# andrewrosemberg/DiffOpt.jl

Measured on AMD Instinct MI355X. Metric: KKT sensitivity solves/sec (fwd+rev) on batched QPs, higher is better.
Workload: dtype f64; 1 GPU; config 2: dense QP batch, fwd+rev sensitivities; problems_per_gpu=1024, n=200, m_ineq=300, p_eq=0, parallelism=batch-sharded x1

## Files before the change

### diffopt.jl_amd/csrc/abi.hip

```cpp
#include <algorithm>
#include <chrono>
#include <cstdlib>
#include <cstring>
#include <initializer_list>

#include "dopt_internal.h"

using dopt::DevBuf;
using dopt::Error;
using dopt::Handle;

struct dopt_handle : public Handle {};

namespace {

template <class F>
int guarded(dopt_handle* h, F&& f) {
  if (!h) return -1;
  try {
    h->err.clear();
    DOPT_CHECK_HIP(hipSetDevice(h->device));
    return f();
  } catch (const Error& e) {
    h->err = e.msg;
// ... 92 lines not shown
  *out = nullptr;
  if (batch < 0 || n < 0 || m < 0 || p < 0 ||
      (kind != DOPT_KIND_QP && kind != DOPT_KIND_CONIC && kind != DOPT_KIND_NLP))
    return -1;
  int ndev = 0;
  if (hipGetDeviceCount(&ndev) != hipSuccess || ndev <= 0) return -4;
  if (device < 0 || device >= ndev) return -1;
  auto* h = new dopt_handle();
  h->device = device;
  h->batch = batch;
  h->n = n;
  h->m = m;
  h->p = p;
  h->kind = kind;
  int rc = guarded(h, [&]() {
    DOPT_CHECK_HIP(hipStreamCreateWithFlags(&h->stream, hipStreamNonBlocking));
    h->own_stream = true;
    if (const char* e = getenv("DOPT_CONIC_SPLIT")) {
      if (e[0] == '0' || e[0] == '1') h->conic_split = e[0] - '0';
    }
    if (const char* e = getenv("DOPT_LU")) h->lu_mode = atoi(e) != 0;
    if (const char* e = getenv("DOPT_SYM")) h->sym_mode = atoi(e) != 0;
    if (const char* e = getenv("DOPT_LEFT")) h->left_mode = atoi(e) != 0;
    if (const char* e = getenv("DOPT_NLP_REDUCE")) h->nlp_reduce = atoi(e) != 0;
    if (const char* e = getenv("DOPT_SPLIT_FUSE")) h->split_fuse = atoi(e) != 0;
    if (kind == DOPT_KIND_QP) {
      if ((int64_t)n + m + p > dopt::DENSE_QP_MAX) {
        h->sparse = true;
        h->kamax.ensure(sizeof(double));
        return 0;
      }
      h->nmax = (int32_t)dopt::round_up(std::max(n + m + p, 1), 32);
      h->ld = h->nmax;
      h->K.ensure((size_t)batch * h->nmax * h->ld * sizeof(double));
      h->ipiv.ensure((size_t)batch * std::max(h->nmax, 1) * sizeof(int32_t));
      h->s.ensure((size_t)batch * std::max(m, 1) * sizeof(double));
      h->kidx.ensure((size_t)2 * batch * std::max(m, 1) * sizeof(int32_t));
      h->kls.ensure((size_t)2 * batch * std::max(m, 1) * sizeof(double));
      h->gk.ensure((size_t)batch * std::max(n, 1) * std::max(m, 1) * sizeof(double));
      h->meta.ensure((size_t)std::max<int64_t>(batch, 1) * sizeof(dopt::QPMeta));
      h->kamax.ensure((size_t)std::max<int64_t>(batch, 1) * sizeof(double));
      h->rhs.ensure((size_t)3 * batch * std::max(h->nmax, 1) * sizeof(double));
      h->x.ensure((size_t)2 * batch * std::max(h->nmax, 1) * sizeof(double));
    }
    return 0;
  });
// ... 63 lines not shown
  });
}

int dopt_set_memory(dopt_handle* h, int32_t mem) {
  return guarded(h, [&]() {
    if (mem != DOPT_MEM_HOST && mem != DOPT_MEM_DEVICE) throw Error(-1, "bad memory mode");
    h->mem = mem;
    return 0;
  });
}

int dopt_set_sparse(dopt_handle* h, int32_t on) {
  return guarded(h, [&]() {
    if (h->kind != DOPT_KIND_QP && h->kind != DOPT_KIND_CONIC) throw Error(-1, "dopt_set_sparse: QP and conic handles only");
    if (h->kind == DOPT_KIND_CONIC) {
      h->sparse = on != 0;
      h->cset = h->cfactored = false;
      return 0;
    }
    if (!on && (int64_t)h->n + h->m + h->p > dopt::DENSE_QP_MAX)
      throw Error(-1, "dopt_set_sparse: n + m + p > 8192 has only the sparse route");
    h->sparse = on != 0;
    h->set = h->factored = h->small_ready = false;
    return 0;
  });
}

int dopt_qp_set(dopt_handle* h, const double* Q, const double* G, const double* hv,
                const double* A, const double* z, const double* lam, const double* nu) {
  return guarded(h, [&]() {
    if (h->kind != DOPT_KIND_QP) throw Error(-1, "dopt_qp_set on a non-QP handle");
    if (h->sparse) throw Error(-1, "dopt_qp_set: a sparse-route handle takes the MOI matrix form (dopt_qp_set_csc)");
    const size_t B = h->batch, n = h->n, m = h->m, p = h->p;
    if (!Q || !z) throw Error(-1, "Q and z are required");
    if (m && (!G || !hv || !lam)) throw Error(-1, "G, h and lam are required when m > 0");
    if (p && (!A || !nu)) throw Error(-1, "A and nu are required when p > 0");
    h->set = false;
    h->factored = false;
    h->small_ready = false;
    h->Q = stage_in(*h, h->own_in[0], Q, B * n * n);
    h->G = m ? stage_in(*h, h->own_in[1], G, B * m * n) : nullptr;
    h->hv = m ? stage_in(*h, h->own_in[2], hv, B * m) : nullptr;
    h->A = p ? stage_in(*h, h->own_in[3], A, B * p * n) : nullptr;
    h->z = stage_in(*h, h->own_in[4], z, B * n);
    h->lam = m ? stage_in(*h, h->own_in[5], lam, B * m) : nullptr;
    h->nu = p ? stage_in(*h, h->own_in[6], nu, B * p) : nullptr;
// ... 1293 lines not shown
```

### diffopt.jl_amd/csrc/dopt_internal.h

```cpp
#pragma once
#include <hip/hip_runtime.h>

#include <cstdint>
#include <functional>
#include <string>
#include <vector>

#include "../../include/diffopt_mi355x.h"

#define DOPT_CHECK_HIP(expr)                                                   \
  do {                                                                         \
    hipError_t _e = (expr);                                                    \
    if (_e != hipSuccess) {                                                    \
      throw dopt::Error(-2, std::string(#expr) + ": " + hipGetErrorString(_e)); \
    }                                                                          \
  } while (0)

namespace dopt {

struct Error {
  int code;
  std::string msg;
  Error(int c, std::string m) : code(c), msg(std::move(m)) {}
};
// ... 116 lines not shown
  DevBuf gk;
  DevBuf dinv;
  DevBuf plist;
  DevBuf glist;
  DevBuf lsqr_ws;
  DevBuf binv;
  hipStream_t aux = nullptr;
  hipEvent_t ev_fork = nullptr, ev_join = nullptr, ev_qsym = nullptr, ev_crit = nullptr;
  hipStream_t crit = nullptr;
  int32_t left_mode = 1;
  DevBuf ukp;
  bool ukp_valid = false;
  bool u_missing = false;
  DevBuf qsy;
  bool qsym_pending = false;
  DevBuf fwdw;
  DevBuf krhs, kx, kfull;
  DevBuf mws;
  QPMeta* meta_host = nullptr;
  hipEvent_t meta_ev = nullptr;
  hipEvent_t meta_fork = nullptr;
  int32_t lu_mode = 1;
  int32_t sym_mode = 1;
  int32_t blocked_npmax = 0;
  bool has_generic = true;
  int32_t n_generic = 0;
  bool info_clear = false;
  bool has_lsqr = true;
  int32_t n_pivot = 0;
  bool set = false, factored = false;
  bool small_ready = false;
  bool sparse = false;
  bool sp_qnz = false;
  SpStore sp[2];
  DevBuf sp_tmp, sp_sort, sp_s, sp_ws, sp_info, sp_rhs;

  const double *cA = nullptr, *cb = nullptr, *cc = nullptr;
  const double *cx = nullptr, *cs = nullptr, *cy = nullptr;
  DevBuf own_cin[6];
  std::vector<int32_t> cones;
  DevBuf cone_dev;
  DevBuf vp, dpi, cwork, cinfo, cnorm;
  DevBuf cinfok;
  int32_t conic_k = 0;
  DevBuf csplit;
  int32_t conic_split = -1;
// ... 58 lines not shown
      DOPT_CHECK_HIP(hipEventElapsedTime(&ms, pe.second.first, pe.second.second));
      phase_ms[pe.first] += ms;
      phase_cnt[pe.first] += 1;
      ev_pool.push_back(pe.second.first);
      ev_pool.push_back(pe.second.second);
    }
    ev_pending.clear();
  }
};

inline void ensure_aux(Handle& h) {
  if (h.aux) return;
  int least = 0, greatest = 0;
  DOPT_CHECK_HIP(hipDeviceGetStreamPriorityRange(&least, &greatest));
  DOPT_CHECK_HIP(hipStreamCreateWithPriority(&h.aux, hipStreamNonBlocking, least));
  DOPT_CHECK_HIP(hipStreamCreateWithPriority(&h.crit, hipStreamNonBlocking, greatest));
  const unsigned fl = hipEventDisableTiming | hipEventReleaseToDevice;
  DOPT_CHECK_HIP(hipEventCreateWithFlags(&h.ev_fork, fl));
  DOPT_CHECK_HIP(hipEventCreateWithFlags(&h.ev_join, fl));
  DOPT_CHECK_HIP(hipEventCreateWithFlags(&h.ev_qsym, fl));
  DOPT_CHECK_HIP(hipEventCreateWithFlags(&h.ev_crit, fl));
  DOPT_CHECK_HIP(hipEventCreateWithFlags(&h.meta_fork, fl));
}
inline double* qsy_max(Handle& h) { return h.qsy.as<double>(); }
inline int32_t* qsy_flag(Handle& h) { return reinterpret_cast<int32_t*>(h.qsy.as<double>() + h.batch); }
inline void qsym_join(Handle& h) {
  if (!h.qsym_pending) return;
  DOPT_CHECK_HIP(hipStreamWaitEvent(h.stream, h.ev_qsym, 0));
  h.qsym_pending = false;
}

struct PhaseTimer {
  Handle& h;
  int phase;
  hipEvent_t e0 = nullptr, e1 = nullptr;
  PhaseTimer(Handle& hh, int ph) : h(hh), phase(ph) {
    if (!(h.prof >> ph & 1u)) return;
    e0 = h.take_event();
    e1 = h.take_event();
    DOPT_CHECK_HIP(hipEventRecord(e0, h.stream));
  }
  ~PhaseTimer() {
    if (!e0) return;
    if (hipEventRecord(e1, h.stream) == hipSuccess) h.ev_pending.push_back({phase, {e0, e1}});
  }
};
// ... 2 lines not shown
bool qp_small_eligible(const Handle& h);
void qp_small_reverse(Handle& h, const double* dl_dz, double* out, int32_t* flags);
void qp_small_forward(Handle& h, const FwdTangents& T, double* out);
void qp_reverse(Handle& h, const double* dl_dz, double* out);
struct CscTriple {
  const int64_t* cp[3];
  const int64_t* rv[3];
  const double* nz[3];
  double* dense[3];
  int rows[3];
};
void csc_to_dense3(Handle& h, const CscTriple& T);
void csc_to_dense(Handle& h, const int64_t* colptr, const int64_t* rowval, const double* nzval,
                  int64_t nnz, int rows, int ncols, double* dense, int* err);
void qp_reverse_grads(Handle& h, const double* rev, double* dQ, double* dq, double* dG, double* gc,
                      double* dA, double* ac);
void qp_forward(Handle& h, const double* dQ, const double* dq, const double* dG,
                const double* dh, const double* dA, const double* db, double* out);
void qp_forward_reverse(Handle& h, const double* dl_dz, const double* dQ,
                        const double* dq, const double* dG, const double* dh,
                        const double* dA, const double* db, double* out_rev,
                        double* out_fwd);
void qp_nopiv_factor(Handle& h, double* dinv, double* w0 = nullptr, double* w1 = nullptr);
void qp_blocked_factor(Handle& h, double* dinv, const int32_t* plist, int count);
void qp_nopiv_materialize_u(Handle& h);
void qp_blocked_solve(Handle& h, const double* dinv, int trans, const double* rhs, double* x, int sel);
void qp_blocked_solve_pair(Handle& h, const double* dinv, const double* rhs0, const double* rhs1, double* x0,
                           double* x1, int sel);
void qp_blocked_solve_multi(Handle& h, const double* dinv, int trans, int k, const double* rhs, double* x,
                            int sel);
void qp_reverse_k(Handle& h, int k, const double* dl_dz, double* out);
void qp_params_reverse(Handle& h, const double* rev, int nparam, int64_t nterms, const int32_t* t_param,
                       const int32_t* t_kind, const int32_t* t_index, const double* t_coef, double* out);
void qp_params_forward(Handle& h, const double* dp, int nparam, int64_t nterms, const int32_t* t_param,
                       const int32_t* t_kind, const int32_t* t_index, const double* t_coef, double* dq,
                       double* dh, double* db);
void qp_forward_k(Handle& h, int k, const double* dQ, const double* dq, const double* dG, const double* dh,
                  const double* dA, const double* db, double* out);
void qp_blocked_solve2(Handle& h, const double* dinv, const double* rhs_rev, const double* rhs_fwd,
                       double* x_rev, double* x_fwd, int sel, const double* w_rev = nullptr,
                       const double* w_fwd = nullptr);
size_t dinv_stride(int nmax);
using ReasmFn = std::function<void(const int32_t*, int)>;
void factor_dense(Handle& h, const ReasmFn& reasm, const std::function<void()>* pre_copy = nullptr,
                  bool* deferred = nullptr);
void factor_dense_finish(Handle& h, const ReasmFn& reasm);
// ... 54 lines not shown
```

### diffopt.jl_amd/csrc/qp.hip

```cpp
#include "device_prims.h"
#include "lsqr_core.h"
#include "qp_assemble.h"

namespace dopt {

constexpr int TPB = 256;
constexpr int OUT_LCAP = 4096;
constexpr int NB = 32;

__global__ __launch_bounds__(TPB) void qp_lu_generic_kernel(
    double* __restrict__ K, int32_t* __restrict__ ipiv, QPMeta* __restrict__ meta,
    int nmax, int ld, const int32_t* __restrict__ plist) {
  __shared__ double redv[4];
  __shared__ int redi[4];
  const int b = plist[blockIdx.x], t = threadIdx.x;
  const int lane = t & 63, wv = t >> 6;
  const int N = meta[b].nsys;
  double* Kb = K + (size_t)b * nmax * ld;
  int32_t* piv = ipiv + (size_t)b * nmax;
  int info = 0;
  for (int j = 0; j < N; ++j) {
    double best = -1.0;
    int bi = 0x7fffffff;
    for (int r = j + t; r < N; r += TPB) {
// ... 192 lines not shown
};

__global__ __launch_bounds__(TPB) void qp_lsqr_kernel(
    const double* __restrict__ K, const QPMeta* __restrict__ meta, int nmax,
    int ld, int trans, const double* __restrict__ rhs, double* __restrict__ xout,
    double* __restrict__ work) {
  __shared__ double red[4];
  const int b = blockIdx.x, t = threadIdx.x;
  if (!meta[b].iterative) return;
  const int N = meta[b].nsys;
  const double* Kb = K + (size_t)b * nmax * ld;
  double* x = work + (size_t)b * 5 * nmax;
  double* u = x + N;
  double* v = u + N;
  double* w = v + N;
  double* tmp = w + N;
  const DenseKKT op{Kb, ld, N, trans};
  LsqrScalars st;
  lsqr_solve<TPB, block_sum>(st, op, rhs + (size_t)b * nmax, 0.0, N, x, u, v, w, tmp, N, red);
  __syncthreads();
  for (int i = t; i < N; i += TPB) xout[(size_t)b * nmax + i] = x[i];
}

__global__ __launch_bounds__(TPB) void qp_rev_rhs_kernel(
    const double* __restrict__ dl_dz, const QPMeta* __restrict__ meta, int n,
    int nmax, double* __restrict__ rhs, double* __restrict__ rhs2) {
  const int b = blockIdx.x, t = threadIdx.x;
  const int N = meta[b].nsys;
  for (int i = t; i < N; i += TPB) {
    const double v = (i < n) ? dl_dz[(size_t)b * n + i] : 0.0;
    rhs[(size_t)b * nmax + i] = v;
    if (rhs2) rhs2[(size_t)b * nmax + i] = v;
  }
}

__global__ __launch_bounds__(TPB) void qp_fwd_rhs_kernel(
    const double* __restrict__ dQ, const double* __restrict__ dq,
    const double* __restrict__ dG, const double* __restrict__ dh,
    const double* __restrict__ dA, const double* __restrict__ db,
    const double* __restrict__ z, const double* __restrict__ lam,
    const double* __restrict__ nu, const int32_t* __restrict__ rpos,
    const QPMeta* __restrict__ meta, int n, int m, int p, int nmax, int zcap,
    double* __restrict__ full, double* __restrict__ rhs, double* __restrict__ rhs2) {
  extern __shared__ __attribute__((aligned(16))) double smem[];
  const int b = blockIdx.x, t = threadIdx.x, lane = t & 63, wv = t >> 6;
  const double* zg = z + (size_t)b * n;
  const double* lb = lam + (size_t)b * m;
  const double* nb = nu + (size_t)b * p;
  const bool staged = n <= zcap;
  if (staged)
    for (int i = t; i < n; i += TPB) smem[i] = zg[i];
  __syncthreads();
  const double* zs = staged ? smem : zg;
  double* r = full + (size_t)b * nmax;
  for (int i = t; i < n; i += TPB) {
    double acc = 0.0;
    if (dQ) {
      const double* Qb = dQ + (size_t)b * n * n;
      for (int j = 0; j < n; ++j) acc = fma(Qb[i + (size_t)j * n], zs[j], acc);
    }
    if (dq) acc += dq[(size_t)b * n + i];
    r[i] = acc;
  }
  __syncthreads();
  if (dG && m > 0) {
    const double* Gb = dG + (size_t)b * m * n;
    for (int i = wv; i < n; i += 4) {
      double acc = 0.0;
// ... 28 lines not shown
      for (int j = 0; j < n; ++j) az = fma(Ab[e + (size_t)j * p], zs[j], az);
    }
    r[n + m + e] = az - (db ? db[(size_t)b * p + e] : 0.0);
  }
  __syncthreads();
  const int nk = meta[b].nk;
  double* rb = rhs + (size_t)b * nmax;
  double* rb2 = rhs2 ? rhs2 + (size_t)b * nmax : nullptr;
  for (int i = t; i < n; i += TPB) {
    rb[i] = r[i];
    if (rb2) rb2[i] = r[i];
  }
  for (int l = t; l < m; l += TPB) {
    const int kk = rpos[(size_t)b * m + l];
    if (kk >= 0) {
      rb[n + kk] = r[n + l];
      if (rb2) rb2[n + kk] = r[n + l];
    }
  }
  for (int e = t; e < p; e += TPB) {
    rb[n + nk + e] = r[n + m + e];
    if (rb2) rb2[n + nk + e] = r[n + m + e];
  }
}

#ifndef DOPT_QP_NT
#define DOPT_QP_NT 0
#endif
__global__ __launch_bounds__(TPB) void qp_output_kernel(
    const double* __restrict__ x0, const double* __restrict__ G,
    const double* __restrict__ s, const int32_t* __restrict__ rpos,
    const QPMeta* __restrict__ meta, const double* __restrict__ full, int n,
    int m, int p, int nmax, int zcap, int trans0, double* __restrict__ out0, const double* __restrict__ x1,
    double* __restrict__ out1, int B) {
  extern __shared__ __attribute__((aligned(16))) double smem[];
  __shared__ int nel;
  const bool second = x1 && (int)blockIdx.x >= B;
  const int b = second ? (int)blockIdx.x - B : (int)blockIdx.x, t = threadIdx.x;
  const double* __restrict__ x = second ? x1 : x0;
  double* __restrict__ out = second ? out1 : out0;
  const int trans = second ? 1 : trans0;
  const int nk = meta[b].nk;
  const double* xb = x + (size_t)b * nmax;
  double* ob = out + (size_t)b * (n + m + p);
  const bool staged = n <= zcap;
  const double* xz = staged ? smem : xb;
// ... 195 lines not shown
static double* dinv_of(Handle& h) {
  h.dinv.ensure((size_t)h.batch * dinv_stride(h.nmax) * sizeof(double));
  return h.dinv.as<double>();
}

static QPIn qp_inputs(Handle& h) {
  static const double dummy = 0.0;
  QPIn P;
  P.Q = h.Q;
  P.G = h.m ? h.G : &dummy;
  P.h = h.m ? h.hv : &dummy;
  P.A = h.p ? h.A : &dummy;
  P.z = h.z;
  P.lam = h.m ? h.lam : &dummy;
  P.nu = h.p ? h.nu : &dummy;
  P.n = h.n;
  P.m = h.m;
  P.p = h.p;
  return P;
}

static int32_t* rpos_of(Handle& h) { return h.kidx.as<int32_t>() + (size_t)h.batch * h.m; }

template <class F>
static void prep_assemble(Handle& h, const int32_t* plist, int count, bool full, F&& after_prep) {
  if (count == 0) return;
  const QPIn P = qp_inputs(h);
  if (!full && h.n > 0) {
    ensure_aux(h);
    h.qsy.ensure((size_t)h.batch * (sizeof(double) + sizeof(int32_t)));
    DOPT_CHECK_HIP(hipEventRecord(h.ev_fork, h.stream));
    DOPT_CHECK_HIP(hipStreamWaitEvent(h.aux, h.ev_fork, 0));
    DOPT_CHECK_HIP(hipMemsetAsync(h.qsy.p, 0, h.qsy.bytes, h.aux));
    hipLaunchKernelGGL(qp_qsym_kernel, dim3((unsigned)qsym_pairs(h.n), (unsigned)count), dim3(256), 0, h.aux, P,
                       qsy_max(h), qsy_flag(h), plist);
    check_launch();
    DOPT_CHECK_HIP(hipEventRecord(h.ev_qsym, h.aux));
    h.qsym_pending = true;
  }
  const dim3 pg(count), pb(prep_threads(h.m));
  if (prep_rows_per_thread(h.m) == 2)
    hipLaunchKernelGGL(qp_prep_kernel<2>, pg, pb, prep_lds(h.n), h.stream, P, h.s.as<double>(),
                       h.kidx.as<int32_t>(), rpos_of(h), h.kls.as<double>(), h.gk.as<double>(), h.batch, h.meta.as<QPMeta>(),
                       plist, h.kamax.as<double>(), h.sym_mode);
  else
    hipLaunchKernelGGL(qp_prep_kernel<1>, pg, pb, prep_lds(h.n), h.stream, P, h.s.as<double>(),
                       h.kidx.as<int32_t>(), rpos_of(h), h.kls.as<double>(), h.gk.as<double>(), h.batch, h.meta.as<QPMeta>(),
                       plist, h.kamax.as<double>(), h.sym_mode);
  check_launch();
  after_prep();
  hipLaunchKernelGGL(qp_asm_tile_kernel, dim3((unsigned)count * ASM_WPP), dim3(512), 0, h.stream, P,
                     h.kidx.as<int32_t>(), h.kls.as<double>(), h.gk.as<double>(), h.batch, h.meta.as<QPMeta>(),
                     h.K.as<double>(), h.ld,
                     h.nmax, plist, full ? 1 : 0, h.kamax.as<double>());
  check_launch();
}
static void prep_assemble(Handle& h, const int32_t* plist, int count) { prep_assemble(h, plist, count, true, [] {}); }

static void meta_copy(Handle& h) {
  if (!h.meta_host) {
    DOPT_CHECK_HIP(hipHostMalloc((void**)&h.meta_host, std::max<size_t>(h.batch, 1) * sizeof(QPMeta)));
    DOPT_CHECK_HIP(hipEventCreateWithFlags(&h.meta_ev, hipEventDisableTiming));
  }
  DOPT_CHECK_HIP(hipMemcpyAsync(h.meta_host, h.meta.p, h.batch * sizeof(QPMeta), hipMemcpyDeviceToHost,
                                h.stream));
  DOPT_CHECK_HIP(hipEventRecord(h.meta_ev, h.stream));
}

static void meta_copy_side(Handle& h) {
  ensure_aux(h);
  if (!h.meta_host) {
    DOPT_CHECK_HIP(hipHostMalloc((void**)&h.meta_host, std::max<size_t>(h.batch, 1) * sizeof(QPMeta)));
    DOPT_CHECK_HIP(hipEventCreateWithFlags(&h.meta_ev, hipEventDisableTiming));
  }
  DOPT_CHECK_HIP(hipEventRecord(h.meta_fork, h.stream));
  DOPT_CHECK_HIP(hipStreamWaitEvent(h.crit, h.meta_fork, 0));
  DOPT_CHECK_HIP(hipMemcpyAsync(h.meta_host, h.meta.p, h.batch * sizeof(QPMeta), hipMemcpyDeviceToHost, h.crit));
  DOPT_CHECK_HIP(hipEventRecord(h.meta_ev, h.crit));
}

static void meta_sizes(Handle& h) {
  DOPT_CHECK_HIP(hipEventSynchronize(h.meta_ev));
  int npmax = 0;
  h.has_generic = h.has_lsqr = false;
  for (int64_t b = 0; b < h.batch; ++b) {
    const QPMeta& mm = h.meta_host[b];
    const int r = qp_route(mm.iterative, mm.nsys);
    if (r == ROUTE_BLOCKED) npmax = std::max(npmax, (mm.nsys + 31) & ~31);
    h.has_generic |= r == ROUTE_GENERIC;
    h.has_lsqr |= r == ROUTE_LSQR;
  }
  h.blocked_npmax = npmax;
}

static int pivot_fallback(Handle& h, const ReasmFn& reasm) {
  DOPT_CHECK_HIP(hipEventSynchronize(h.meta_ev));
  std::vector<int32_t> list;
  for (int64_t b = 0; b < h.batch; ++b)
    if (h.meta_host[b].lu == LU_REJECT && ((h.meta_host[b].nsys + 31) & ~31) <= PIVOT_MAX)
      list.push_back((int32_t)b);
  const int count = (int)list.size();
  if (count) {
    h.plist.ensure(list.size() * sizeof(int32_t));
    DOPT_CHECK_HIP(hipMemcpyAsync(h.plist.p, list.data(), list.size() * sizeof(int32_t),
                                  hipMemcpyHostToDevice, h.stream));
    const int32_t* pl = h.plist.as<int32_t>();
    reasm(pl, count);
    qp_blocked_factor(h, dinv_of(h), pl, count);
    DOPT_CHECK_HIP(hipStreamSynchronize(h.stream));
  }
  return count;
}

static void generic_lu(Handle& h, const std::vector<int32_t>& list) {
  h.n_generic = (int)list.size();
// ... 21 lines not shown
    }
    if (any) {
      PhaseTimer pt(h, DOPT_PHASE_QP_LU_PIVOT);
      h.n_pivot = pivot_fallback(h, reasm);
    }
    if (!big.empty()) {
      h.plist.ensure(big.size() * sizeof(int32_t));
      DOPT_CHECK_HIP(hipMemcpyAsync(h.plist.p, big.data(), big.size() * sizeof(int32_t), hipMemcpyHostToDevice,
                                    h.stream));
      reasm(h.plist.as<int32_t>(), (int)big.size());
      DOPT_CHECK_HIP(hipStreamSynchronize(h.stream));
      glist.insert(glist.end(), big.begin(), big.end());
    }
  }
  h.n_generic = 0;
  if (!glist.empty()) {
    PhaseTimer pt(h, DOPT_PHASE_QP_LU_PIVOT);
    generic_lu(h, glist);
  }
}

template <class F>
static void factor_blocked(Handle& h, F&& spec, double* w0, double* w1, const ReasmFn& reasm,
                           const std::function<void()>* pre_copy = nullptr, bool* deferred = nullptr) {
  auto np_of = [](const QPMeta& mm) { return (mm.nsys + 31) & ~31; };
  std::vector<int32_t> glist;
  if (h.has_generic)
    for (int64_t b = 0; b < h.batch; ++b) {
      const QPMeta& mm = h.meta_host[b];
      if (qp_route(mm.iterative, mm.nsys) == ROUTE_GENERIC) glist.push_back((int32_t)b);
    }
  if (deferred) *deferred = false;
  if (h.lu_mode == 1) {
    {
      PhaseTimer pt(h, DOPT_PHASE_QP_LU);
      qp_nopiv_factor(h, dinv_of(h), w0, w1);
    }
    if (pre_copy) (*pre_copy)();
    if (h.blocked_npmax) meta_copy_side(h);
    spec();
    h.n_pivot = 0;
    if (deferred && h.blocked_npmax && glist.empty()) {
      *deferred = true;
      return;
    }
    factor_blocked_rest(h, reasm, glist, true);
  } else {
    {
      PhaseTimer pt(h, DOPT_PHASE_QP_LU_PIVOT);
      qp_blocked_factor(h, dinv_of(h), nullptr, (int)h.batch);
    }
    spec();
    h.n_pivot = -1;
    if (h.blocked_npmax > PIVOT_MAX)
      for (int64_t b = 0; b < h.batch; ++b) {
        const QPMeta& mm = h.meta_host[b];
        if (qp_route(mm.iterative, mm.nsys) == ROUTE_BLOCKED && np_of(mm) > PIVOT_MAX) glist.push_back((int32_t)b);
// ... 85 lines not shown
static void finish_pair(Handle& h, double* out_rev, double* out_fwd) {
  finish_into(h, 1, rhs_of(h, 1), x_of(h, 1), full_of(h), nullptr, nullptr, nullptr, true);
  finish_into(h, 0, rhs_of(h, 0), x_of(h, 0), full_of(h), out_rev, x_of(h, 1), out_fwd);
}

static void rev_rhs(Handle& h, const double* dl_dz, double* copy = nullptr) {
  PhaseTimer pt(h, DOPT_PHASE_QP_RHS);
  hipLaunchKernelGGL(qp_rev_rhs_kernel, dim3(h.batch), dim3(TPB), 0, h.stream, dl_dz, h.meta.as<QPMeta>(),
                     h.n, h.nmax, rhs_of(h, 0), copy);
  check_launch();
}

static void fwd_rhs_into(Handle& h, const FwdTangents& T, double* full, double* rhs, double* copy = nullptr) {
  const int B = (int)h.batch, n = h.n, m = h.m, p = h.p;
  static const double dummy = 0.0;
  hipLaunchKernelGGL(qp_fwd_rhs_kernel, dim3(B), dim3(TPB), (size_t)std::min(n, ZCAP) * sizeof(double),
                     h.stream, T.dQ, T.dq, T.dG, T.dh, T.dA, T.db, h.z, m ? h.lam : &dummy,
                     p ? h.nu : &dummy, rpos_of(h), h.meta.as<QPMeta>(), n, m, p, h.nmax, ZCAP, full, rhs, copy);
  check_launch();
}
static void fwd_rhs(Handle& h, const FwdTangents& T, double* copy = nullptr) {
  PhaseTimer pt(h, DOPT_PHASE_QP_RHS);
  fwd_rhs_into(h, T, full_of(h), rhs_of(h, 1), copy);
}

static FwdTangents tangents(Handle& h, const double* dQ, const double* dq, const double* dG,
                            const double* dh, const double* dA, const double* db) {
  FwdTangents T;
  T.dQ = dQ;
  T.dq = dq;
  T.dG = h.m ? dG : nullptr;
  T.dh = h.m ? dh : nullptr;
  T.dA = h.p ? dA : nullptr;
  T.db = h.p ? db : nullptr;
  return T;
}

void qp_reverse(Handle& h, const double* dl_dz, double* out) {
  if (!h.factored) qp_factor(h);
  rev_rhs(h, dl_dz);
  {
    PhaseTimer pt(h, DOPT_PHASE_QP_SOLVE);
    qp_blocked_solve(h, dinv_of(h), 0, rhs_of(h, 0), x_of(h, 0), LU_SEL_ALL);
  }
  finish(h, 0, out);
}
// ... 88 lines not shown
  }
  solve_k(h, 1, k, rk, xk, fk, out);
}

void qp_reverse_grads(Handle& h, const double* rev, double* dQ, double* dq, double* dG, double* gc,
                      double* dA, double* ac) {
  if (!h.set) throw Error(-1, "dopt_qp_reverse_grads: dopt_qp_set has not been called");
  static const double dummy = 0.0;
  const long long per = (long long)h.n * h.n + (long long)(h.m + h.p) * h.n + h.n + h.m + h.p;
  const int gx = (int)std::max<long long>(1, std::min<long long>((per + TPB - 1) / TPB, 64));
  const int gy = (int)std::min<int64_t>(h.batch, 65535);
  hipLaunchKernelGGL(qp_reverse_grads_kernel, dim3(gx, gy), dim3(TPB), 0, h.stream, rev, h.z,
                     h.m ? h.lam : &dummy, h.p ? h.nu : &dummy, (int)h.batch, h.n, h.m, h.p, dQ, dq,
                     h.m ? dG : nullptr, h.m ? gc : nullptr, h.p ? dA : nullptr, h.p ? ac : nullptr);
  check_launch();
}

void qp_forward_reverse(Handle& h, const double* dl_dz, const double* dQ,
                        const double* dq, const double* dG, const double* dh,
                        const double* dA, const double* db, double* out_rev,
                        double* out_fwd) {
  if (!h.set) throw Error(-1, "dopt_qp_forward_reverse: dopt_qp_set has not been called");
  const FwdTangents T = tangents(h, dQ, dq, dG, dh, dA, db);
  {
    PhaseTimer pt(h, DOPT_PHASE_QP_ASSEMBLE);
    prep_assemble(h, nullptr, (int)h.batch, h.lu_mode == 0, [&] { meta_copy_side(h); });
  }
  double *w0 = nullptr, *w1 = nullptr;
  if (h.lu_mode == 1) {
    const size_t len = (size_t)h.batch * h.nmax;
    h.fwdw.ensure(2 * len * sizeof(double));
    w0 = h.fwdw.as<double>();
    w1 = w0 + len;
  }
  rev_rhs(h, dl_dz, w0);
  fwd_rhs(h, T, w1);
  meta_sizes(h);
  if (!h.blocked_npmax) w0 = w1 = nullptr;
  auto solve2 = [&](int sel, const double* sw0, const double* sw1) {
    PhaseTimer pt(h, DOPT_PHASE_QP_SOLVE);
    qp_blocked_solve2(h, dinv_of(h), rhs_of(h, 0), rhs_of(h, 1), x_of(h, 0), x_of(h, 1), sel, sw0, sw1);
  };
  const bool spec_out = h.lu_mode == 1 && !h.has_generic && !h.has_lsqr;
  h.n_generic = 0;
  factor_blocked(
      h,
      [&] {
        solve2(h.lu_mode == 1 ? LU_SEL_NOPIV : LU_SEL_ALL, w0, w1);
        if (spec_out) finish_pair(h, out_rev, out_fwd);
      },
      w0, w1, qp_reasm(h));
  if (h.n_pivot > 0) solve2(LU_SEL_PIVOT, nullptr, nullptr);
  if (!spec_out || h.n_pivot > 0 || h.n_generic > 0) finish_pair(h, out_rev, out_fwd);
  h.factored = true;
  h.info_clear = h.lu_mode == 1 && h.n_pivot == 0 && h.n_generic == 0;
}

}
```

### diffopt.jl_amd/csrc/qp_nopiv.hip

```cpp
#include "device_prims.h"
#include "nlp_defs.h"

#ifndef NLU_STOP
#define NLU_STOP 99
#endif
#ifndef NLU_ROT
#define NLU_ROT (blockIdx.x & 3)
#endif
#ifdef NLU_STAMPS
__device__ unsigned long long nlu_stamps[16];
#define NLU_MARK(k)                                                              \
  do {                                                                          \
    if (threadIdx.x == 0) {                                                     \
      const unsigned long long now_ = __builtin_amdgcn_s_memtime();             \
      atomicAdd(&nlu_stamps[k], now_ - st_last_);                               \
      st_last_ = now_;                                                          \
    }                                                                           \
  } while (0)
#define NLU_MARK_INIT unsigned long long st_last_ = __builtin_amdgcn_s_memtime()
#else
#define NLU_MARK(k) do {} while (0)
#define NLU_MARK_INIT do {} while (0)
#endif
#ifdef LDIAG_STAMPS
// ... 1343 lines not shown
        if (j < t) acc = fma(S[t * SLD + j], P[j] * vec[j], acc);
      if (t < Wv) w0b[c0 + t] = fma(acc, RP[t], vec[t]);
    } else if (t < 128) {
      const int j = t - 64;
      double acc = vec[64 + j];
#pragma unroll 8
      for (int i = 0; i < NB64; ++i)
        if (i < j) acc = fma(vec[64 + i], S[j * SLD + i], acc);
      if (j < Wv) w1b[c0 + j] = acc * P[j] * RD[j];
    }
  }
  LD_MARK(10);
}

template <class SRC>
__device__ __forceinline__ void ldiag_body(
    double* S, int b, double* __restrict__ K, int ld, int nmax, int32_t* __restrict__ perm,
    double* __restrict__ dinv, size_t dstride, QPMeta* __restrict__ meta, int c0, double* __restrict__ binv,
    double* __restrict__ ukp, double* __restrict__ w0, double* __restrict__ w1, double* __restrict__ kamax,
    const double* __restrict__ kls, int n, int m, const SRC& src) {
  LD_MARK(0);
  const QPMeta mm = meta[b];
  const int Np = nlu_np(mm);
  if (c0 >= Np || mm.lu == LU_REJECT) return;
  const int Wv = min(NB64, Np - c0);
  const int t = threadIdx.x, lane = t & 63, wv = t >> 6, g = lane >> 4, l16 = lane & 15;
  double* Kb = K + (size_t)b * nmax * ld;
  const auto sv = src_bind(src, b, mm);
  const PScale ps = pscale(kls, b, n, m, mm);
  double* ud = ukp + (size_t)b * nmax;
  double* w0b = w0 ? w0 + (size_t)b * nmax : nullptr;
  double* w1b = w0 ? w1 + (size_t)b * nmax : nullptr;
  double amax = __hip_atomic_load(kamax + b, __ATOMIC_RELAXED, __HIP_MEMORY_SCOPE_AGENT);
  if (c0 == 0) {
    if (src.qflag) {
      if (src.qflag[b]) {
        if (t == 0) meta[b].lu = LU_REJECT;
        return;
      }
      amax = fmax(amax, src.qmax[b]);
      if (t == 0) kamax[b] = amax;
    }
  }
  d4 accd[3];
#pragma unroll
  for (int q = 0; q < 3; ++q) accd[q] = (d4){0, 0, 0, 0};
  double sweep = 0.0;
// ... 125 lines not shown
  const int oq = c * n + r, og = c * v.m + rn, oa = c * v.p + (rn - nk);
  int off = cq ? (rq ? oq : (rg ? og : oa)) : rn;
  const double* base = cq ? (rq ? v.Q : (rg ? v.gk : v.A)) : v.sk;
  off = live ? off : 0;
  base = live ? base : v.Q;
  p = base + off;
  return live ? 1 : 0;
}
__device__ __forceinline__ int src_ref_tile(const NSrcB& v, const double* X, int r, int c, int ri, int ci,
                                            const double*& p) {
  const int* tc = lc_codes(X);
  return nlp_R_ref_lower(v.s->d, v.s->in, v.s->R, v.b, r, c, tc[ri], tc[64 + ci], p);
}

template <class SRC>
__device__ __forceinline__ void lcol_body(double* X, int b, int it, double* __restrict__ K, int ld, int nmax,
                                          QPMeta* __restrict__ meta, int c0, const double* __restrict__ binv,
                                          const double* __restrict__ ukp, int cnt,
                                          const double* __restrict__ kamax, const double* __restrict__ kls, int n,
                                          int m, const SRC& src) {
  const QPMeta mm = meta[b];
  const int Np = nlu_np(mm);
  const int r0 = c0 + NB64 + 64 * it;
  if (mm.lu == LU_REJECT || it >= cnt || r0 >= Np) return;
  const int sw = min(NB64, Np - r0);
  const int t = threadIdx.x, lane = t & 63, wv = t >> 6, g = lane >> 4, l16 = lane & 15;
  const bool wact = 16 * wv < sw;
  double* Kb = K + (size_t)b * nmax * ld;
  const double* ud = ukp + (size_t)b * nmax;
  const double* Bg = binv + (size_t)b * BSTR;
  const auto sv = src_bind(src, b, mm);
  const PScale ps = pscale(kls, b, n, m, mm);
  const int rho = lane >> 3, gam = lane & 7;
  auto issue = [&](int st) {
    double* buf = X + (st & 1) * LC_STAGE;
    const int ks = 16 * st;
#pragma unroll
    for (int q = 0; q < 2; ++q) {
      const int c = 2 * wv + q, r = 8 * c + rho, col = ks + 2 * (gam ^ ((r >> 1) & 7));
      const int rt = r < sw ? r0 + r : r0;
      glds16(Kb + (size_t)rt * ld + col, buf + c * 128);
      glds16(Kb + (size_t)(c0 + r) * ld + col, buf + LC_IMG + c * 128);
    }
    if (wv == 0) glds16(ud + ks + 2 * gam, X + LC_DS + (st & 1) * 128);
  };
  auto issue_uinv = [&]() {
    const int hr = lane >> 5, gq = lane & 31;
// ... 162 lines not shown

__global__ __launch_bounds__(256) void nlu_sym_uinv_kernel(double* __restrict__ dinv, size_t dstride,
                                                           const QPMeta* __restrict__ meta,
                                                           const double* __restrict__ ukp, int nmax,
                                                           const double* __restrict__ kls, int n, int m) {
  const int b = blockIdx.y, kb = blockIdx.x;
  const QPMeta mm = meta[b];
  if (mm.lu != LU_NOPIV || !mm.sym) return;
  const int Np = nlu_np(mm);
  if (32 * kb >= Np) return;
  double* D = dinv + (size_t)b * dstride + (size_t)kb * DBLK;
  const double* ud = ukp + (size_t)b * nmax + 32 * kb;
  const PScale ps = pscale(kls, b, n, m, mm);
  for (int e = threadIdx.x; e < 32 * 32; e += 256) {
    const int i = e >> 5, j = e & 31;
    D[32 * 32 + e] = i <= j ? D[j * 32 + i] / (ps(32 * kb + i) * ud[j]) : 0.0;
  }
}

}

template <class SRC>
static void left_lu(Handle& h, const SRC& src, double* dinv, double* w0, double* w1, const double* kls,
                    double* kamax) {
  const int npmax = h.blocked_npmax;
  const int B = (int)h.batch;
  const size_t dstride = dinv_stride(h.nmax);
  double* K = h.K.as<double>();
  int32_t* perm = h.ipiv.as<int32_t>();
  QPMeta* meta = h.meta.as<QPMeta>();
  h.binv.ensure((size_t)2 * B * BSTR * sizeof(double));
  h.ukp.ensure((size_t)B * h.nmax * sizeof(double));
  h.ukp_valid = true;
  h.u_missing = true;
  double* ukp = h.ukp.as<double>();
  hipStream_t S = h.stream;
  auto binv_of = [&](int c0) { return h.binv.as<double>() + (size_t)((c0 / NB64) & 1) * B * BSTR; };
  for (int c0 = 0; c0 < npmax; c0 += NB64) {
    double* bv = binv_of(c0);
    hipLaunchKernelGGL((nlu_ldiag_kernel<SRC>), dim3(B), dim3(PNT), 0, S, K, h.ld, h.nmax, perm, dinv, dstride, meta,
                       c0, bv, ukp, w0, w1, kamax, kls, h.n, h.m, src, 0);
    DOPT_CHECK_HIP(hipGetLastError());
    const int ntile = (npmax - c0 - NB64 + 63) / 64;
    if (ntile <= 0) break;
    const long long tot = (long long)ntile * B;
    if (tot > 0x7fffffffLL) throw Error(-1, "no-pivot LU: grid too large");
    hipLaunchKernelGGL((nlu_lcol_kernel<SRC>), dim3((unsigned)tot), dim3(256), 0, S, K, h.ld, h.nmax, meta, c0, bv,
                       ukp, ntile, (int)tot, kamax, kls, h.n, h.m, src);
    DOPT_CHECK_HIP(hipGetLastError());
  }
}

void qp_nopiv_factor(Handle& h, double* dinv, double* w0, double* w1) {
  qsym_join(h);
  h.ukp_valid = false;
  h.u_missing = false;
  const int npmax = h.blocked_npmax;
  if (npmax == 0) return;
  const int B = (int)h.batch;
  const bool qp = h.kind == DOPT_KIND_QP;
  const double* kls = qp ? h.kls.as<double>() : nullptr;
  double* kamax = h.kamax.as<double>();
  int lower = qp && h.meta_host ? 1 : 0;
  static const double zero = 0.0;
  QSrc src;
  src.Q = qp ? h.Q : &zero;
  src.gk = qp ? h.gk.as<double>() : &zero;
  src.kls = qp ? h.kls.as<double>() : &zero;
  src.A = qp && h.p ? h.A : &zero;
  const bool qchk = qp && h.qsy.p && h.n > 0;
  src.qmax = qchk ? qsy_max(h) : nullptr;
  src.qflag = qchk ? qsy_flag(h) : nullptr;
  src.n = h.n;
  src.m = h.m;
  src.p = h.p;
  src.B = h.batch;
  const int srcmode = qp ? 1 : 0;
  if (lower)
    for (int64_t b = 0; b < h.batch; ++b) {
      const QPMeta& mm = h.meta_host[b];
      if (qp_route(mm.iterative, mm.nsys) == ROUTE_BLOCKED && !mm.sym) {
        lower = 0;
        break;
      }
    }
  const size_t dstride = dinv_stride(h.nmax);
  double* K = h.K.as<double>();
  int32_t* perm = h.ipiv.as<int32_t>();
  QPMeta* meta = h.meta.as<QPMeta>();
  if (h.kind == DOPT_KIND_NLP && h.nlp_left) {
    NSrc ns;
    ns.d = nlp_dims(h);
    ns.in = nlp_inputs(h);
    ns.R = nlp_red_of(h);
    ns.qmax = qsy_max(h);
    ns.qflag = qsy_flag(h);
    left_lu(h, ns, dinv, w0, w1, nullptr, kamax);
    return;
  }
  if (lower && h.left_mode) {
    left_lu(h, src, dinv, w0, w1, kls, kamax);
    return;
  }
  h.binv.ensure((size_t)2 * B * BSTR * sizeof(double));
  auto binv_of = [&](int c) { return h.binv.as<double>() + (size_t)((c / NB64) & 1) * B * BSTR; };
  auto grid = [](long long g) {
    if (g > 0x7fffffffLL) throw Error(-1, "no-pivot LU: grid too large");
    return dim3((unsigned)g);
  };
  hipStream_t S = h.stream, T = h.stream;
  if (lower) {
    ensure_aux(h);
    T = h.aux;
    if (h.crit) {
      S = h.crit;
      DOPT_CHECK_HIP(hipEventRecord(h.ev_crit, h.stream));
      DOPT_CHECK_HIP(hipStreamWaitEvent(S, h.ev_crit, 0));
    }
  }
  auto fork = [&] {
    DOPT_CHECK_HIP(hipEventRecord(h.ev_fork, S));
    DOPT_CHECK_HIP(hipStreamWaitEvent(T, h.ev_fork, 0));
  };
  auto join = [&] {
// ... 93 lines not shown
```

Before: 904,800 solves/s.

## Speculatively launch left-looking LU before host metadata scan using prior call's size

Records the padded system size and symmetry status from previous forward+reverse calls. On later calls it queues prep, a fused forward/reverse RHS kernel, and the left-looking no-pivot LU before the host synchronises on the metadata copy, so the host wait no longer serialises the factor launch. If the scan shows the guess was wrong or a system is non-symmetric, it synchronises all streams and redoes the normal path. The separate rev/fwd RHS launches are also merged into one kernel with a 2B grid. This risks wasted work on misprediction and relies on the LU kernels skipping non-symmetric systems.

Result: no change. 908,400 solves/s, median of 6 (+0.4%).

```diff
diff --git a/diffopt.jl_amd/csrc/abi.hip b/diffopt.jl_amd/csrc/abi.hip
--- a/diffopt.jl_amd/csrc/abi.hip
+++ b/diffopt.jl_amd/csrc/abi.hip
@@ -138,6 +138,7 @@
     if (const char* e = getenv("DOPT_LU")) h->lu_mode = atoi(e) != 0;
     if (const char* e = getenv("DOPT_SYM")) h->sym_mode = atoi(e) != 0;
     if (const char* e = getenv("DOPT_LEFT")) h->left_mode = atoi(e) != 0;
+    if (const char* e = getenv("DOPT_LU_SPEC")) h->lu_spec = atoi(e) != 0;
     if (const char* e = getenv("DOPT_NLP_REDUCE")) h->nlp_reduce = atoi(e) != 0;
     if (const char* e = getenv("DOPT_SPLIT_FUSE")) h->split_fuse = atoi(e) != 0;
     if (kind == DOPT_KIND_QP) {
@@ -247,6 +248,7 @@
       throw Error(-1, "dopt_set_sparse: n + m + p > 8192 has only the sparse route");
     h->sparse = on != 0;
     h->set = h->factored = h->small_ready = false;
+    dopt::spec_drop(*h);
     return 0;
   });
 }
diff --git a/diffopt.jl_amd/csrc/dopt_internal.h b/diffopt.jl_amd/csrc/dopt_internal.h
--- a/diffopt.jl_amd/csrc/dopt_internal.h
+++ b/diffopt.jl_amd/csrc/dopt_internal.h
@@ -162,6 +162,9 @@
   hipEvent_t meta_fork = nullptr;
   int32_t lu_mode = 1;
   int32_t sym_mode = 1;
+  int32_t lu_spec = 1;
+  int32_t spec_np[4] = {0, 0, 0, 0};
+  bool spec_qual = false;
   int32_t blocked_npmax = 0;
   bool has_generic = true;
   int32_t n_generic = 0;
@@ -266,6 +269,10 @@
   DOPT_CHECK_HIP(hipEventCreateWithFlags(&h.ev_crit, fl));
   DOPT_CHECK_HIP(hipEventCreateWithFlags(&h.meta_fork, fl));
 }
+inline void spec_drop(Handle& h) {
+  for (int32_t& v : h.spec_np) v = 0;
+  h.spec_qual = false;
+}
 inline double* qsy_max(Handle& h) { return h.qsy.as<double>(); }
 inline int32_t* qsy_flag(Handle& h) { return reinterpret_cast<int32_t*>(h.qsy.as<double>() + h.batch); }
 inline void qsym_join(Handle& h) {
@@ -314,6 +321,7 @@
                         const double* dA, const double* db, double* out_rev,
                         double* out_fwd);
 void qp_nopiv_factor(Handle& h, double* dinv, double* w0 = nullptr, double* w1 = nullptr);
+void qp_nopiv_left_spec(Handle& h, double* dinv, double* w0, double* w1, int npmax);
 void qp_blocked_factor(Handle& h, double* dinv, const int32_t* plist, int count);
 void qp_nopiv_materialize_u(Handle& h);
 void qp_blocked_solve(Handle& h, const double* dinv, int trans, const double* rhs, double* x, int sel);
diff --git a/diffopt.jl_amd/csrc/qp.hip b/diffopt.jl_amd/csrc/qp.hip
--- a/diffopt.jl_amd/csrc/qp.hip
+++ b/diffopt.jl_amd/csrc/qp.hip
@@ -238,10 +238,10 @@
   for (int i = t; i < N; i += TPB) xout[(size_t)b * nmax + i] = x[i];
 }
 
-__global__ __launch_bounds__(TPB) void qp_rev_rhs_kernel(
-    const double* __restrict__ dl_dz, const QPMeta* __restrict__ meta, int n,
+__device__ __forceinline__ void rev_rhs_body(
+    int b, const double* __restrict__ dl_dz, const QPMeta* __restrict__ meta, int n,
     int nmax, double* __restrict__ rhs, double* __restrict__ rhs2) {
-  const int b = blockIdx.x, t = threadIdx.x;
+  const int t = threadIdx.x;
   const int N = meta[b].nsys;
   for (int i = t; i < N; i += TPB) {
     const double v = (i < n) ? dl_dz[(size_t)b * n + i] : 0.0;
@@ -249,17 +249,21 @@
     if (rhs2) rhs2[(size_t)b * nmax + i] = v;
   }
 }
-
-__global__ __launch_bounds__(TPB) void qp_fwd_rhs_kernel(
-    const double* __restrict__ dQ, const double* __restrict__ dq,
+__global__ __launch_bounds__(TPB) void qp_rev_rhs_kernel(
+    const double* __restrict__ dl_dz, const QPMeta* __restrict__ meta, int n,
+    int nmax, double* __restrict__ rhs, double* __restrict__ rhs2) {
+  rev_rhs_body(blockIdx.x, dl_dz, meta, n, nmax, rhs, rhs2);
+}
+
+__device__ __forceinline__ void fwd_rhs_body(
+    int b, double* smem, const double* __restrict__ dQ, const double* __restrict__ dq,
     const double* __restrict__ dG, const double* __restrict__ dh,
     const double* __restrict__ dA, const double* __restrict__ db,
     const double* __restrict__ z, const double* __restrict__ lam,
     const double* __restrict__ nu, const int32_t* __restrict__ rpos,
     const QPMeta* __restrict__ meta, int n, int m, int p, int nmax, int zcap,
     double* __restrict__ full, double* __restrict__ rhs, double* __restrict__ rhs2) {
-  extern __shared__ __attribute__((aligned(16))) double smem[];
-  const int b = blockIdx.x, t = threadIdx.x, lane = t & 63, wv = t >> 6;
+  const int t = threadIdx.x, lane = t & 63, wv = t >> 6;
   const double* zg = z + (size_t)b * n;
   const double* lb = lam + (size_t)b * m;
   const double* nb = nu + (size_t)b * p;
@@ -334,6 +338,38 @@
     rb[n + nk + e] = r[n + m + e];
     if (rb2) rb2[n + nk + e] = r[n + m + e];
   }
+}
+__global__ __launch_bounds__(TPB) void qp_fwd_rhs_kernel(
+    const double* __restrict__ dQ, const double* __restrict__ dq,
+    const double* __restrict__ dG, const double* __restrict__ dh,
+    const double* __restrict__ dA, const double* __restrict__ db,
+    const double* __restrict__ z, const double* __restrict__ lam,
+    const double* __restrict__ nu, const int32_t* __restrict__ rpos,
+    const QPMeta* __restrict__ meta, int n, int m, int p, int nmax, int zcap,
+    double* __restrict__ full, double* __restrict__ rhs, double* __restrict__ rhs2) {
+  extern __shared__ __attribute__((aligned(16))) double smem[];
+  fwd_rhs_body(blockIdx.x, smem, dQ, dq, dG, dh, dA, db, z, lam, nu, rpos, meta, n, m, p, nmax, zcap, full, rhs,
+               rhs2);
+}
+
+struct RevRhsArgs {
+  const double* dl_dz;
+  double *rhs, *rhs2;
+};
+__global__ __launch_bounds__(TPB) void qp_rhs_pair_kernel(
+    const double* __restrict__ dQ, const double* __restrict__ dq,
+    const double* __restrict__ dG, const double* __restrict__ dh,
+    const double* __restrict__ dA, const double* __restrict__ db,
+    const double* __restrict__ z, const double* __restrict__ lam,
+    const double* __restrict__ nu, const int32_t* __restrict__ rpos,
+    const QPMeta* __restrict__ meta, int n, int m, int p, int nmax, int zcap,
+    double* __restrict__ full, double* __restrict__ rhs, double* __restrict__ rhs2, RevRhsArgs R, int B) {
+  extern __shared__ __attribute__((aligned(16))) double smem[];
+  const int b = blockIdx.x;
+  if (b < B)
+    fwd_rhs_body(b, smem, dQ, dq, dG, dh, dA, db, z, lam, nu, rpos, meta, n, m, p, nmax, zcap, full, rhs, rhs2);
+  else
+    rev_rhs_body(b - B, R.dl_dz, meta, n, nmax, R.rhs, R.rhs2);
 }
 
 #ifndef DOPT_QP_NT
@@ -575,22 +611,20 @@
 
 static int32_t* rpos_of(Handle& h) { return h.kidx.as<int32_t>() + (size_t)h.batch * h.m; }
 
-template <class F>
-static void prep_assemble(Handle& h, const int32_t* plist, int count, bool full, F&& after_prep) {
-  if (count == 0) return;
-  const QPIn P = qp_inputs(h);
-  if (!full && h.n > 0) {
-    ensure_aux(h);
-    h.qsy.ensure((size_t)h.batch * (sizeof(double) + sizeof(int32_t)));
-    DOPT_CHECK_HIP(hipEventRecord(h.ev_fork, h.stream));
-    DOPT_CHECK_HIP(hipStreamWaitEvent(h.aux, h.ev_fork, 0));
-    DOPT_CHECK_HIP(hipMemsetAsync(h.qsy.p, 0, h.qsy.bytes, h.aux));
-    hipLaunchKernelGGL(qp_qsym_kernel, dim3((unsigned)qsym_pairs(h.n), (unsigned)count), dim3(256), 0, h.aux, P,
-                       qsy_max(h), qsy_flag(h), plist);
-    check_launch();
-    DOPT_CHECK_HIP(hipEventRecord(h.ev_qsym, h.aux));
-    h.qsym_pending = true;
-  }
+static void queue_qsym(Handle& h, const QPIn& P, const int32_t* plist, int count) {
+  ensure_aux(h);
+  h.qsy.ensure((size_t)h.batch * (sizeof(double) + sizeof(int32_t)));
+  DOPT_CHECK_HIP(hipEventRecord(h.ev_fork, h.stream));
+  DOPT_CHECK_HIP(hipStreamWaitEvent(h.aux, h.ev_fork, 0));
+  DOPT_CHECK_HIP(hipMemsetAsync(h.qsy.p, 0, h.qsy.bytes, h.aux));
+  hipLaunchKernelGGL(qp_qsym_kernel, dim3((unsigned)qsym_pairs(h.n), (unsigned)count), dim3(256), 0, h.aux, P,
+                     qsy_max(h), qsy_flag(h), plist);
+  check_launch();
+  DOPT_CHECK_HIP(hipEventRecord(h.ev_qsym, h.aux));
+  h.qsym_pending = true;
+}
+
+static void queue_prep(Handle& h, const QPIn& P, const int32_t* plist, int count) {
   const dim3 pg(count), pb(prep_threads(h.m));
   if (prep_rows_per_thread(h.m) == 2)
     hipLaunchKernelGGL(qp_prep_kernel<2>, pg, pb, prep_lds(h.n), h.stream, P, h.s.as<double>(),
@@ -601,6 +635,14 @@
                        h.kidx.as<int32_t>(), rpos_of(h), h.kls.as<double>(), h.gk.as<double>(), h.batch, h.meta.as<QPMeta>(),
                        plist, h.kamax.as<double>(), h.sym_mode);
   check_launch();
+}
+
+template <class F>
+static void prep_assemble(Handle& h, const int32_t* plist, int count, bool full, F&& after_prep) {
+  if (count == 0) return;
+  const QPIn P = qp_inputs(h);
+  if (!full && h.n > 0) queue_qsym(h, P, plist, count);
+  queue_prep(h, P, plist, count);
   after_prep();
   hipLaunchKernelGGL(qp_asm_tile_kernel, dim3((unsigned)count * ASM_WPP), dim3(512), 0, h.stream, P,
                      h.kidx.as<int32_t>(), h.kls.as<double>(), h.gk.as<double>(), h.batch, h.meta.as<QPMeta>(),
@@ -632,18 +674,41 @@
   DOPT_CHECK_HIP(hipEventRecord(h.meta_ev, h.crit));
 }
 
-static void meta_sizes(Handle& h) {
+struct MetaScan {
+  int npmax = 0;
+  bool generic = false, lsqr = false;
+  bool sym = true;
+};
+static MetaScan meta_scan(Handle& h) {
   DOPT_CHECK_HIP(hipEventSynchronize(h.meta_ev));
-  int npmax = 0;
-  h.has_generic = h.has_lsqr = false;
+  MetaScan s;
   for (int64_t b = 0; b < h.batch; ++b) {
     const QPMeta& mm = h.meta_host[b];
     const int r = qp_route(mm.iterative, mm.nsys);
-    if (r == ROUTE_BLOCKED) npmax = std::max(npmax, (mm.nsys + 31) & ~31);
-    h.has_generic |= r == ROUTE_GENERIC;
-    h.has_lsqr |= r == ROUTE_LSQR;
-  }
-  h.blocked_npmax = npmax;
+    if (r == ROUTE_BLOCKED) s.npmax = std::max(s.npmax, (mm.nsys + 31) & ~31);
+    s.generic |= r == ROUTE_GENERIC;
+    s.lsqr |= r == ROUTE_LSQR;
+    s.sym &= r == ROUTE_BLOCKED && mm.sym != 0;
+  }
+  return s;
+}
+static void meta_apply(Handle& h, const MetaScan& s) {
+  h.has_generic = s.generic;
+  h.has_lsqr = s.lsqr;
+  h.blocked_npmax = s.npmax;
+}
+static void meta_sizes(Handle& h) { meta_apply(h, meta_scan(h)); }
+
+static int spec_guess(const Handle& h) {
+  if (h.kind != DOPT_KIND_QP || h.lu_mode != 1 || !h.left_mode || !h.sym_mode || !h.lu_spec || h.n <= 0) return 0;
+  if (!h.spec_qual) return 0;
+  return *std::max_element(h.spec_np, h.spec_np + 4);
+}
+static void spec_record(Handle& h, const MetaScan& s) {
+  if (!s.sym || s.npmax == 0) return spec_drop(h);
+  for (int i = 3; i > 0; --i) h.spec_np[i] = h.spec_np[i - 1];
+  h.spec_np[0] = s.npmax;
+  h.spec_qual = true;
 }
 
 static int pivot_fallback(Handle& h, const ReasmFn& reasm) {
@@ -711,7 +776,8 @@
 
 template <class F>
 static void factor_blocked(Handle& h, F&& spec, double* w0, double* w1, const ReasmFn& reasm,
-                           const std::function<void()>* pre_copy = nullptr, bool* deferred = nullptr) {
+                           const std::function<void()>* pre_copy = nullptr, bool* deferred = nullptr,
+                           bool lu_queued = false) {
   auto np_of = [](const QPMeta& mm) { return (mm.nsys + 31) & ~31; };
   std::vector<int32_t> glist;
   if (h.has_generic)
@@ -721,7 +787,7 @@
     }
   if (deferred) *deferred = false;
   if (h.lu_mode == 1) {
-    {
+    if (!lu_queued) {
       PhaseTimer pt(h, DOPT_PHASE_QP_LU);
       qp_nopiv_factor(h, dinv_of(h), w0, w1);
     }
@@ -853,6 +919,18 @@
 static void fwd_rhs(Handle& h, const FwdTangents& T, double* copy = nullptr) {
   PhaseTimer pt(h, DOPT_PHASE_QP_RHS);
   fwd_rhs_into(h, T, full_of(h), rhs_of(h, 1), copy);
+}
+
+static void rhs_pair(Handle& h, const double* dl_dz, const FwdTangents& T, double* w0, double* w1) {
+  PhaseTimer pt(h, DOPT_PHASE_QP_RHS);
+  const int B = (int)h.batch, n = h.n, m = h.m, p = h.p;
+  if (B == 0) return;
+  static const double dummy = 0.0;
+  const RevRhsArgs R{dl_dz, rhs_of(h, 0), w0};
+  hipLaunchKernelGGL(qp_rhs_pair_kernel, dim3(2 * (unsigned)B), dim3(TPB), (size_t)std::min(n, ZCAP) * sizeof(double),
+                     h.stream, T.dQ, T.dq, T.dG, T.dh, T.dA, T.db, h.z, m ? h.lam : &dummy, p ? h.nu : &dummy,
+                     rpos_of(h), h.meta.as<QPMeta>(), n, m, p, h.nmax, ZCAP, full_of(h), rhs_of(h, 1), w1, R, B);
+  check_launch();
 }
 
 static FwdTangents tangents(Handle& h, const double* dQ, const double* dq, const double* dG,
@@ -987,10 +1065,6 @@
                         double* out_fwd) {
   if (!h.set) throw Error(-1, "dopt_qp_forward_reverse: dopt_qp_set has not been called");
   const FwdTangents T = tangents(h, dQ, dq, dG, dh, dA, db);
-  {
-    PhaseTimer pt(h, DOPT_PHASE_QP_ASSEMBLE);
-    prep_assemble(h, nullptr, (int)h.batch, h.lu_mode == 0, [&] { meta_copy_side(h); });
-  }
   double *w0 = nullptr, *w1 = nullptr;
   if (h.lu_mode == 1) {
     const size_t len = (size_t)h.batch * h.nmax;
@@ -998,9 +1072,42 @@
     w0 = h.fwdw.as<double>();
     w1 = w0 + len;
   }
-  rev_rhs(h, dl_dz, w0);
-  fwd_rhs(h, T, w1);
-  meta_sizes(h);
+  bool hit = false;
+  if (const int guess = spec_guess(h)) {
+    {
+      PhaseTimer pt(h, DOPT_PHASE_QP_ASSEMBLE);
+      const QPIn P = qp_inputs(h);
+      queue_qsym(h, P, nullptr, (int)h.batch);
+      queue_prep(h, P, nullptr, (int)h.batch);
+    }
+    rhs_pair(h, dl_dz, T, w0, w1);
+    meta_copy_side(h);
+    {
+      PhaseTimer pt(h, DOPT_PHASE_QP_LU);
+      qp_nopiv_left_spec(h, dinv_of(h), w0, w1, guess);
+    }
+    const MetaScan s = meta_scan(h);
+    hit = s.sym && s.npmax > 0 && s.npmax <= guess;
+    if (hit) {
+      meta_apply(h, s);
+      spec_record(h, s);
+    } else {
+      DOPT_CHECK_HIP(hipStreamSynchronize(h.stream));
+      DOPT_CHECK_HIP(hipStreamSynchronize(h.aux));
+      DOPT_CHECK_HIP(hipStreamSynchronize(h.crit));
+      spec_drop(h);
+    }
+  }
+  if (!hit) {
+    {
+      PhaseTimer pt(h, DOPT_PHASE_QP_ASSEMBLE);
+      prep_assemble(h, nullptr, (int)h.batch, h.lu_mode == 0, [&] { meta_copy_side(h); });
+    }
+    rhs_pair(h, dl_dz, T, w0, w1);
+    const MetaScan s = meta_scan(h);
+    meta_apply(h, s);
+    spec_record(h, s);
+  }
   if (!h.blocked_npmax) w0 = w1 = nullptr;
   auto solve2 = [&](int sel, const double* sw0, const double* sw1) {
     PhaseTimer pt(h, DOPT_PHASE_QP_SOLVE);
@@ -1014,7 +1121,7 @@
         solve2(h.lu_mode == 1 ? LU_SEL_NOPIV : LU_SEL_ALL, w0, w1);
         if (spec_out) finish_pair(h, out_rev, out_fwd);
       },
-      w0, w1, qp_reasm(h));
+      w0, w1, qp_reasm(h), nullptr, nullptr, hit);
   if (h.n_pivot > 0) solve2(LU_SEL_PIVOT, nullptr, nullptr);
   if (!spec_out || h.n_pivot > 0 || h.n_generic > 0) finish_pair(h, out_rev, out_fwd);
   h.factored = true;
diff --git a/diffopt.jl_amd/csrc/qp_nopiv.hip b/diffopt.jl_amd/csrc/qp_nopiv.hip
--- a/diffopt.jl_amd/csrc/qp_nopiv.hip
+++ b/diffopt.jl_amd/csrc/qp_nopiv.hip
@@ -1389,7 +1389,7 @@
   LD_MARK(0);
   const QPMeta mm = meta[b];
   const int Np = nlu_np(mm);
-  if (c0 >= Np || mm.lu == LU_REJECT) return;
+  if (c0 >= Np || mm.lu == LU_REJECT || !mm.sym) return;
   const int Wv = min(NB64, Np - c0);
   const int t = threadIdx.x, lane = t & 63, wv = t >> 6, g = lane >> 4, l16 = lane & 15;
   double* Kb = K + (size_t)b * nmax * ld;
@@ -1561,7 +1561,7 @@
   const QPMeta mm = meta[b];
   const int Np = nlu_np(mm);
   const int r0 = c0 + NB64 + 64 * it;
-  if (mm.lu == LU_REJECT || it >= cnt || r0 >= Np) return;
+  if (mm.lu == LU_REJECT || !mm.sym || it >= cnt || r0 >= Np) return;
   const int sw = min(NB64, Np - r0);
   const int t = threadIdx.x, lane = t & 63, wv = t >> 6, g = lane >> 4, l16 = lane & 15;
   const bool wact = 16 * wv < sw;
@@ -1770,8 +1770,7 @@
 
 template <class SRC>
 static void left_lu(Handle& h, const SRC& src, double* dinv, double* w0, double* w1, const double* kls,
-                    double* kamax) {
-  const int npmax = h.blocked_npmax;
+                    double* kamax, int npmax) {
   const int B = (int)h.batch;
   const size_t dstride = dinv_stride(h.nmax);
   double* K = h.K.as<double>();
@@ -1799,17 +1798,8 @@
   }
 }
 
-void qp_nopiv_factor(Handle& h, double* dinv, double* w0, double* w1) {
-  qsym_join(h);
-  h.ukp_valid = false;
-  h.u_missing = false;
-  const int npmax = h.blocked_npmax;
-  if (npmax == 0) return;
-  const int B = (int)h.batch;
+static QSrc qp_src(Handle& h) {
   const bool qp = h.kind == DOPT_KIND_QP;
-  const double* kls = qp ? h.kls.as<double>() : nullptr;
-  double* kamax = h.kamax.as<double>();
-  int lower = qp && h.meta_host ? 1 : 0;
   static const double zero = 0.0;
   QSrc src;
   src.Q = qp ? h.Q : &zero;
@@ -1823,6 +1813,26 @@
   src.m = h.m;
   src.p = h.p;
   src.B = h.batch;
+  return src;
+}
+
+void qp_nopiv_left_spec(Handle& h, double* dinv, double* w0, double* w1, int npmax) {
+  qsym_join(h);
+  left_lu(h, qp_src(h), dinv, w0, w1, h.kls.as<double>(), h.kamax.as<double>(), npmax);
+}
+
+void qp_nopiv_factor(Handle& h, double* dinv, double* w0, double* w1) {
+  qsym_join(h);
+  h.ukp_valid = false;
+  h.u_missing = false;
+  const int npmax = h.blocked_npmax;
+  if (npmax == 0) return;
+  const int B = (int)h.batch;
+  const bool qp = h.kind == DOPT_KIND_QP;
+  const double* kls = qp ? h.kls.as<double>() : nullptr;
+  double* kamax = h.kamax.as<double>();
+  int lower = qp && h.meta_host ? 1 : 0;
+  const QSrc src = qp_src(h);
   const int srcmode = qp ? 1 : 0;
   if (lower)
     for (int64_t b = 0; b < h.batch; ++b) {
@@ -1843,11 +1853,11 @@
     ns.R = nlp_red_of(h);
     ns.qmax = qsy_max(h);
     ns.qflag = qsy_flag(h);
-    left_lu(h, ns, dinv, w0, w1, nullptr, kamax);
+    left_lu(h, ns, dinv, w0, w1, nullptr, kamax, npmax);
     return;
   }
   if (lower && h.left_mode) {
-    left_lu(h, src, dinv, w0, w1, kls, kamax);
+    left_lu(h, src, dinv, w0, w1, kls, kamax, npmax);
     return;
   }
   h.binv.ensure((size_t)2 * B * BSTR * sizeof(double));
```
